# woolgathering/pyPeriod

Measured on AMD Instinct MI355X. Metric: window-projections/sec (all-p sweep, N=4096), higher is better.
Workload: dtype f64

## Files before the change

### pyperiod_amd/csrc/ph_mbest.h

```cpp
#pragma once

#include "ph_device.h"
#include "ph_pair.h"

namespace ph {

__device__ __forceinline__ bool skip_test(const uint32_t* skip, int i) { return (skip[i >> 5] >> (i & 31)) & 1u; }
__device__ __forceinline__ void skip_set(uint32_t* skip, int i) { skip[i >> 5] |= 1u << (i & 31); }

template <typename Norm>
__device__ __forceinline__ bool mbest_prefers(double ss, int p, double best_ss, int bestp, int gamma, Norm&& norm) {
  bool take = bestp == 0;
  if (!take) {
    const double lhs = gamma ? ss * (double)bestp : ss;
    const double rhs = gamma ? best_ss * (double)p : best_ss;
    if (lhs > rhs * (1.0 + 1e-14)) {
      take = true;
    } else if (lhs >= rhs * (1.0 - 1e-14)) {
      const double vn = norm(ss, gamma ? p : 0);
      const double vb = norm(best_ss, gamma ? bestp : 0);
      take = vn > vb || (vn == vb && p < bestp);
    }
  }
  return take;
}

__device__ __forceinline__ int mbest_book(int& row, int bestp, double best, int p_lo, int tid, int& filled, int& repeats,
                                          double* norms, uint32_t* periods, uint32_t* skip) {
  int action;
  __syncthreads();
  if (row >= 0 && repeats < 10) {
    action = 2;
    if (tid == 0) norms[row] += best;
    repeats += 1;
  } else if (row >= 0) {
    action = 0;
    if (tid == 0) skip_set(skip, bestp - p_lo);
    repeats = 0;
  } else {
    action = 1;
    row = filled;
    if (tid == 0) {
      periods[row] = (uint32_t)bestp;
      norms[row] = best;
    }
    filled += 1;
    repeats = 0;
  }
  return action;
}

template <typename T, bool LW>
__global__ __launch_bounds__(1024) __attribute__((amdgpu_waves_per_eu(PH_STEP1_WAVES, 8))) void k_mbest_step1(const T* __restrict__ x, int N, int num, int p_lo,
                                                        int p_hi, int gamma, unsigned flags, Tables tb,
                                                        const PGeom* __restrict__ geom,
                                                        const PassPlan* __restrict__ plan, int n_pass,
                                                        T* __restrict__ gbuf, T* gwin,
                                                        int max_iters, uint32_t* __restrict__ periods_out,
                                                        double* __restrict__ norms_out, T* __restrict__ rows_out,
                                                        int row_stride, double* __restrict__ dnorm_out,
                                                        int* __restrict__ status_out,
                                                        int* __restrict__ sweeps_out, int small_means) {
  extern __shared__ __attribute__((aligned(16))) unsigned char smem[];
  Carve cv(smem);
  T* work = window_buf<T, LW>(cv, gwin, N + kPad);
  const bool general = flags & (kTrunc | kOrth);
  T* buf = !general ? nullptr : gbuf ? gbuf + (int64_t)blockIdx.x * N : cv.take<T>(N);
  double* red = cv.take<double>(kRedDoubles);
  double* wbest = cv.take<double>(kMaxWaves);
  int* wbestp = cv.take<int>(kMaxWaves);
  double* norms = cv.take<double>(num);
  uint32_t* periods = cv.take<uint32_t>(num);
  const int P = p_hi - p_lo + 1;
  uint32_t* skip = cv.take<uint32_t>((P + 31) / 32);
  T* msm = small_means ? cv.take<T>(kPairSmallP) : nullptr;
  T* prt = small_means ? cv.take<T>(kPairSplitW) : nullptr;

  const int64_t w = blockIdx.x;
  const int tid = threadIdx.x;
  const int lane = tid & (kWave - 1);
  const int wv = __builtin_amdgcn_readfirstlane(tid >> 6);
  const int nw = blockDim.x >> 6;
  T* rows = rows_out + w * (int64_t)num * row_stride;

  load_window(x + w * (int64_t)N, work, N);
  zero_pad(work, N);
  for (int k = tid; k < num; k += blockDim.x) {
    norms[k] = 0.0;
    periods[k] = 0u;
  }
  for (int k = tid; k < (P + 31) / 32; k += blockDim.x) skip[k] = 0u;
  __syncthreads();
  const double data_norm = uniform_f64(periodic_norm_from_sq(block_sumsq(work, N, red), N, 0));

  int filled = 0;
  int repeats = 0;
  int status = 0;
  int iters = 0;
  while (filled < num) {
    if (++iters > max_iters) {
      status = 2;
      break;
    }
    double best = 0.0;
    int bestp = 0;
    if (!general) {
      double best_ss = 0.0;
      wave_sweep_plan<T, LW>(work, N, geom, plan, wv, n_pass, nw, lane, [&](double ss, int p) {
        if (skip_test(skip, p - p_lo) || !(ss > 0.0)) return;
        bool take = bestp == 0;
        if (!take) {
          const double lhs = gamma ? ss * (double)bestp : ss;
          const double rhs = gamma ? best_ss * (double)p : best_ss;
          if (lhs > rhs * (1.0 + 1e-14)) {
            take = true;
          } else if (lhs >= rhs * (1.0 - 1e-14)) {
            const double vn = periodic_norm_from_sq(ss, N, gamma ? p : 0);
            const double vb = periodic_norm_from_sq(best_ss, N, gamma ? bestp : 0);
            take = vn > vb || (vn == vb && p < bestp);
          }
        }
        if (take) {
          best_ss = ss;
          bestp = p;
        }
      });
      best = bestp != 0 ? periodic_norm_from_sq(best_ss, N, gamma ? bestp : 0) : 0.0;
      if (!(best > 0.0)) bestp = 0;
      wave_argmax(best, bestp);
      if (lane == 0) {
        wbest[wv] = best;
        wbestp[wv] = bestp;
      }
      __syncthreads();
      red_argmax(wbest, wbestp, nw, best, bestp);
      __syncthreads();
    } else {
      for (int p = p_lo; p <= p_hi; ++p) {
        const double v = block_sweep_value(work, buf, N, p, gamma ? p : 0, flags, tb, red);
        if (v > best && !skip_test(skip, p - p_lo)) {
          best = v;
          bestp = p;
        }
      }
    }
    if (bestp == 0) {
      status = 1;
      break;
    }
    int row = -1;
    for (int k = 0; k < num; ++k)
      if (periods[k] == (uint32_t)bestp) row = k;
    int action;
    __syncthreads();
    if (row >= 0 && repeats < 10) {
      action = 2;
      if (tid == 0) norms[row] += best;
      repeats += 1;
    } else if (row >= 0) {
      action = 0;
      if (tid == 0) skip_set(skip, bestp - p_lo);
      repeats = 0;
    } else {
      action = 1;
      row = filled;
      if (tid == 0) {
        periods[row] = (uint32_t)bestp;
        norms[row] = best;
      }
      filled += 1;
      repeats = 0;
    }
    T* brow = rows + (int64_t)(row < 0 ? 0 : row) * row_stride;
    if (!general && msm && bestp <= kPairSmallP) {
      split_row_means(work, msm, prt, N, bestp, tid, min((int)blockDim.x, kPairSplitW));
      if (tid < bestp) {
        const T m = msm[tid];
        if (action == 1)
          brow[tid] = m;
        else if (action == 2)
          brow[tid] += m;
      }
      int idx = tid % bestp;
      const int step = blockDim.x % bestp;
      for (int n = tid; n < N; n += blockDim.x) {
        work[n] -= msm[idx];
        idx += step;
        idx = idx >= bestp ? idx - bestp : idx;
      }
    } else if (!general) {
      const Fold f(N, bestp);
      for (int j = tid; j < bestp; j += blockDim.x) {
        const T m = residue_mean(work, f, j, false);
        const int cnt = f.count(j);
        if (action == 1)
          brow[j] = m;
        else if (action == 2)
          brow[j] += m;
        for (int r = 0; r < cnt; ++r) work[r * bestp + j] -= m;
      }
    } else {
      project_lds(work, buf, N, bestp, flags, tb);
      for (int n = tid; n < N; n += blockDim.x) {
        const T m = buf[n];
        if (n < bestp) {
          if (action == 1)
            brow[n] = m;
          else if (action == 2)
            brow[n] += m;
        }
        work[n] -= m;
      }
    }
    __syncthreads();
  }
  __syncthreads();
  for (int k = tid; k < num; k += blockDim.x) {
    periods_out[w * num + k] = periods[k];
    norms_out[w * num + k] = norms[k];
  }
  if (tid == 0) {
    dnorm_out[w] = data_norm;
    status_out[w] = status;
    if (sweeps_out) sweeps_out[w] = status == 2 ? iters - 1 : iters;
  }
}

constexpr int kPairCoop = 6;

enum {
  MP_LISTED = 0,
  MP_FILLED = 2,
  MP_REPEATS = 4,
  MP_STATUS = 6,
  MP_SWEEPS = 8,
  MP_RUNNING = 10,
  MP_EXACT_ALL = 12,
  MP_QUEUE = 14,
  MP_WORDS = 16
};
enum { MP_UNIT = 0, MP_SCALE = 2, MP_DOUBLES = 4 };

__device__ __forceinline__ double pair_exact_part(const double* __restrict__ xs, int p, const PGeom& g, int first, int stride) {
  double part = 0.0;
  for (int j = first; j < p; j += stride) {
    const bool full = j < g.nfull;
    const double s = column_sum(xs, j, p, full ? g.rows : g.rows - 1);
    part = fma(s * s, full ? g.w_full : g.w_short, part);
  }
  return part;
}

__global__ __launch_bounds__(1024) __attribute__((amdgpu_waves_per_eu(PH_STEP1_WAVES, 8))) void k_mbest_step1_pair(
    const double* __restrict__ x, int W, int N, int num, int p_lo, int p_hi, int p_scr, int gamma,
    const int* __restrict__ fac_off, const int* __restrict__ fac_q, const PGeom* __restrict__ geom, const PGeomF* __restrict__ geomf, const double* __restrict__ radq, const PassPlan* __restrict__ plan, int n_pass,
    double* __restrict__ gres, int max_iters, uint32_t* __restrict__ periods_out, double* __restrict__ norms_out,
    double* __restrict__ rows_out, int row_stride, double* __restrict__ dnorm_out, int* __restrict__ status_out,
    int* __restrict__ sweeps_out) {
  extern __shared__ __attribute__((aligned(16))) unsigned char smem[];
  Carve cv(smem);
  f2* pw = cv.take<f2>(N + kPad);
  double* stg = cv.take<double>(N + kPad);
  double* red = cv.take<double>(kRedDoubles);
  double* wbest = cv.take<double>(kMaxWaves);
  int* wbestp = cv.take<int>(kMaxWaves);
  double* norms = cv.take<double>(2 * num);
  uint32_t* periods = cv.take<uint32_t>(2 * num);
  const int P = p_hi - p_lo + 1;
  const int SK = (P + 31) / 32;
  uint32_t* skip = cv.take<uint32_t>(2 * SK);
  int* list = cv.take<int>(2 * kPairListCap);
  int* ctl = cv.take<int>(MP_WORDS);
  double* dst2 = cv.take<double>(MP_DOUBLES);
  double* msm = cv.take<double>(kPairSmallP);
  double* prt = cv.take<double>(kPairSplitW);

  const int tid = threadIdx.x;
  const int wv = __builtin_amdgcn_readfirstlane(tid >> 6);
  const int nw = blockDim.x >> 6;
  const size_t gstride = win_stride((size_t)N);
  float* pwf = reinterpret_cast<float*>(pw);
  const double sqrtN = uniform_f64(sqrt((double)N));

  for (int k = tid; k < 2 * num; k += blockDim.x) {
    norms[k] = 0.0;
    periods[k] = 0u;
  }
  for (int k = tid; k < 2 * SK; k += blockDim.x) skip[k] = 0u;
  if (tid < MP_WORDS) ctl[tid] = tid == MP_QUEUE ? nw : 0;
  zero_pad(stg, N);
  for (int i = tid; i < kPad; i += blockDim.x) pw[N + i] = f2_zero();
  for (int w = 0; w < 2; ++w) {
    const int64_t gw = 2 * (int64_t)blockIdx.x + w;
    const bool exists = gw < W;
    __syncthreads();
    if (exists) {
      load_window(x + gw * (int64_t)N, stg, N);
    } else {
      for (int n = tid; n < N; n += blockDim.x) stg[n] = 0.0;
    }
    __syncthreads();
    const double rsq = block_sumsq(stg, N, red);
    const double sc = uniform_f64(pair_pick_scale(rsq, N));
    for (int n = tid; n < N; n += blockDim.x) pwf[2 * n + w] = (float)(stg[n] * sc);
    if (tid == 0) {
      dst2[MP_UNIT + w] = rsq * sc * sc * (1.0 + 1e-9);
      dst2[MP_SCALE + w] = sc;
      ctl[MP_RUNNING + w] = exists ? 1 : 0;
      ctl[MP_EXACT_ALL + w] = pair_usable(rsq) ? 0 : 1;
      if (exists) dnorm_out[gw] = periodic_norm_from_sq_n(rsq, sqrtN, 0);
    }
  }
  StageClock<kPairTimers, 5, 2> clk;
  WgStamp<kClocks> stamp;
  for (;;) {
    __syncthreads();
    const bool act0 = __builtin_amdgcn_readfirstlane(ctl[MP_RUNNING]) != 0, act1 = __builtin_amdgcn_readfirstlane(ctl[MP_RUNNING + 1]) != 0;
    if (!act0 && !act1) break;
    prio_by_progress(__builtin_amdgcn_readfirstlane(max(ctl[MP_SWEEPS], ctl[MP_SWEEPS + 1])));
    if (wv == 0 && pair_lane() == 0) ctl[MP_LISTED] = ctl[MP_LISTED + 1] = 0;
    f2* vals = reinterpret_cast<f2*>(stg);
    pair_sweep_plan<false, true>(
        pw, N, geomf, plan, wv, n_pass, nw, [&](float z, int q) { pair_store1(vals, z, q, p_lo); },
        [&](float z, int q_a, int q_b) { pair_store2(vals, z, q_a, q_b, p_lo); },
        PH_PAIR_QUEUE ? &ctl[MP_QUEUE] : nullptr);
    __syncthreads();
    clk.mark(0);
    prio_short_phase();
    {
    const int tid = (wv << 6) + pair_lane();
    const int lane = tid & (kWave - 1);
    if (tid == 0) ctl[MP_QUEUE] = nw;
    {
      const bool scr0 = act0 && !__builtin_amdgcn_readfirstlane(ctl[MP_EXACT_ALL]), scr1 = act1 && !__builtin_amdgcn_readfirstlane(ctl[MP_EXACT_ALL + 1]);
      if (scr0 || scr1) {
        const double unit0 = uniform_f64(dst2[MP_UNIT]), unit1 = uniform_f64(dst2[MP_UNIT + 1]);
        const int i0 = p_scr - p_lo;
        const bool cover = i0 > 0;
        const int SD = (i0 + 31) >> 5;
        uint32_t* seen = reinterpret_cast<uint32_t*>(stg);
        for (int k = tid; k < 2 * SD; k += blockDim.x) seen[k] = 0u;
        const double slack = cover ? pair_cover_slack(N) : 0.0;
        struct Entry {
          f2 v;
          double rad, rq;
          bool skip0, skip1;
        };
        auto entry = [&](int idx) {
          Entry e;
          const int q = p_lo + idx;
          const uint32_t bit = 1u << (idx & 31);
          e.v = vals[idx];
          e.rad = radq[q];
          e.rq = gamma ? 1.0 / (double)q : 1.0;
          e.skip0 = (skip[idx >> 5] & bit) != 0;
          e.skip1 = (skip[SK + (idx >> 5)] & bit) != 0;
          return e;
        };
        const int idx_own = i0 + tid;
        Entry own = {f2_zero(), 0.0, 1.0, true, true};
        if (idx_own < P) own = entry(idx_own);
        double lo0 = -1.0 / 0.0, lo1 = -1.0 / 0.0;
        for (int idx = idx_own; idx < P; idx += blockDim.x) {
          const Entry e = idx == idx_own ? own : entry(idx);
          double a = (double)e.v.x - e.rad * unit0, b = (double)e.v.y - e.rad * unit1;
          if (gamma) {
            a *= e.rq;
            b *= e.rq;
          }
          if (!e.skip0 && a > lo0) lo0 = a;
          if (!e.skip1 && b > lo1) lo1 = b;
        }
        lo0 = wave_max(lo0);
        lo1 = wave_max(lo1);
        if (lane == 0) {
          red[wv] = lo0;
          red[kMaxWaves + wv] = lo1;
        }
        __syncthreads();
        lo0 = uniform_f64(red_combine<true>(red, nw));
        lo1 = uniform_f64(red_combine<true>(red + kMaxWaves, nw));
        const bool none0 = cover && scr0 && !(lo0 > -1.0 / 0.0), none1 = cover && scr1 && !(lo1 > -1.0 / 0.0);
        if (tid == 0 && none0) ctl[MP_LISTED] = kPairListCap + 1;
        if (tid == 0 && none1) ctl[MP_LISTED + 1] = kPairListCap + 1;
        const double thr0 = lo0 - fabs(lo0) * 1e-9, thr1 = lo1 - fabs(lo1) * 1e-9;
        for (int idx = idx_own; idx < P; idx += blockDim.x) {
          const Entry e = idx == idx_own ? own : entry(idx);
          const int q = p_lo + idx;
          const double rad = e.rad + slack;
          double a = (double)e.v.x + rad * unit0, b = (double)e.v.y + rad * unit1;
          if (gamma) {
            a *= e.rq;
            b *= e.rq;
          }
          const bool hit0 = scr0 && !none0 && a >= thr0, hit1 = scr1 && !none1 && b >= thr1;
          if (hit0 && !e.skip0) {
            const int k = atomicAdd(&ctl[MP_LISTED], 1);
            if (k < kPairListCap) list[k] = q;
          }
          if (hit1 && !e.skip1) {
            const int k = atomicAdd(&ctl[MP_LISTED + 1], 1);
            if (k < kPairListCap) list[kPairListCap + k] = q;
          }
          if (cover && (hit0 || hit1)) {
            const int f1 = fac_off[q + 1];
            for (int f = fac_off[q] - (p_lo == 1 ? 1 : 0); f < f1; ++f) {
              const int d = f < fac_off[q] ? 1 : fac_q[f];
              if (d < p_lo || d >= p_scr) continue;
              const int di = d - p_lo;
              const uint32_t dbit = 1u << (di & 31);
              for (int w = 0; w < 2; ++w) {
                if (!(w ? hit1 : hit0) || (skip[w * SK + (di >> 5)] & dbit)) continue;
                if (atomicOr(&seen[w * SD + (di >> 5)], dbit) & dbit) continue;
                const int k = atomicAdd(&ctl[MP_LISTED + w], 1);
                if (k < kPairListCap) list[w * kPairListCap + k] = d;
              }
            }
          }
        }
      }
    }
    __syncthreads();
    clk.mark(1);
    for (int w = 0; w < 2; ++w) {
      if (!(w ? act1 : act0)) continue;
      const int64_t gw = 2 * (int64_t)blockIdx.x + w;
      int filled = __builtin_amdgcn_readfirstlane(ctl[MP_FILLED + w]), repeats = __builtin_amdgcn_readfirstlane(ctl[MP_REPEATS + w]), status = 0,
          iters = __builtin_amdgcn_readfirstlane(ctl[MP_SWEEPS + w]);
      const int nlisted = __builtin_amdgcn_readfirstlane(ctl[MP_LISTED + w]);
      const bool exact_all = __builtin_amdgcn_readfirstlane(ctl[MP_EXACT_ALL + w]) != 0 || nlisted > kPairListCap;
      int ncand = exact_all ? P : nlisted;
      double* nrm = norms + w * num;
      uint32_t* per = periods + w * num;
      uint32_t* sk = skip + w * SK;
      const int* lst = list + w * kPairListCap;
      __syncthreads();
      if (iters + 1 > max_iters) {
        status = 2;
      } else {
        const double* src = iters == 0 ? x + gw * (int64_t)N : gres + gw * gstride;
        iters += 1;
        load_window(src, stg, N);
        __syncthreads();
        clk.mark(2);
        if (kPairTimers) {
          clk.count(0, ncand);
          clk.count(1, exact_all ? 1 : 0);
        }
        if (p_scr > p_lo && !exact_all && ncand > 1) {
          for (int k = wv; k < ncand; k += nw) {
            const int p = lst[k];
            const PGeom g = geom[p];
            const double part = p < 64 ? wave_partial_small(stg, N, p, g, lane) : pair_exact_part(stg, p, g, lane, kWave);
            const double ss = wave_sum(part);
            if (lane == 0) msm[k] = ss;
          }
          __syncthreads();
          if (wv == 0) {
            const int k0 = lane, k1 = kWave + lane;
            const double v0 = k0 < ncand ? msm[k0] : -1.0, v1 = k1 < ncand ? msm[k1] : -1.0;
            const int q0 = lst[k0], q1 = k1 < kPairListCap ? lst[k1] : 0;
            const double top = wave_max(fmax(v0, v1));
            const bool keep0 = k0 < ncand && v0 >= top - fabs(top) * 1e-9, keep1 = k1 < ncand && v1 >= top - fabs(top) * 1e-9;
            const unsigned long long m0 = __ballot(keep0), m1 = __ballot(keep1);
            const unsigned long long below = (1ull << lane) - 1ull;
            const int n0 = __popcll(m0);
            int* out = list + w * kPairListCap;
            if (keep0) out[__popcll(m0 & below)] = q0;
            if (keep1) out[n0 + __popcll(m1 & below)] = q1;
            if (lane == 0) ctl[MP_LISTED + w] = n0 + __popcll(m1);
          }
          __syncthreads();
          ncand = __builtin_amdgcn_readfirstlane(ctl[MP_LISTED + w]);
        }
        double best_ss = 0.0;
        int bestp = 0;
        const auto norm = [&](double s, int div) { return periodic_norm_from_sq_n(s, sqrtN, div); };
        auto consider = [&](double ss, int p) {
          if (!(ss > 0.0)) return;
          if (mbest_prefers(ss, p, best_ss, bestp, gamma, norm)) {
            best_ss = ss;
            bestp = p;
          }
        };
        double best = 0.0;
        if (ncand <= kPairCoop) {
          for (int k = 0; k < ncand; ++k) {
            const int p = exact_all ? p_lo + k : lst[k];
            if (skip_test(sk, p - p_lo)) continue;
            const PGeom g = geom[p];
            double part = 0.0;
            if (p < 64) {
              if (wv == 0) part = wave_partial_small(stg, N, p, g, lane);
            } else {
              part = pair_exact_part(stg, p, g, tid, blockDim.x);
            }
            consider(block_sum(part, red), p);
          }
          best = bestp != 0 ? periodic_norm_from_sq_n(best_ss, sqrtN, gamma ? bestp : 0) : 0.0;
          if (!(best > 0.0)) bestp = 0;
        } else {
          for (int k = wv; k < ncand; k += nw) {
            const int p = exact_all ? p_lo + k : lst[k];
            if (skip_test(sk, p - p_lo)) continue;
            const PGeom g = geom[p];
            const double part = p < 64 ? wave_partial_small(stg, N, p, g, lane) : pair_exact_part(stg, p, g, lane, kWave);
            consider(wave_sum(part), p);
          }
          best = bestp != 0 ? periodic_norm_from_sq_n(best_ss, sqrtN, gamma ? bestp : 0) : 0.0;
          if (!(best > 0.0)) bestp = 0;
          if (lane == 0) {
            wbest[wv] = best;
            wbestp[wv] = bestp;
          }
          __syncthreads();
          red_argmax(wbest, wbestp, nw, best, bestp);
          __syncthreads();
        }
        clk.mark(3);
        if (bestp == 0) {
          status = 1;
        } else {
          int row = -1;
          for (int k0 = 0; k0 < num; k0 += kWave) {
            const unsigned long long hit = __ballot(k0 + lane < num && per[k0 + lane] == (uint32_t)bestp);
            if (hit) row = k0 + 63 - __clzll(hit);
          }
          const int action = mbest_book(row, bestp, best, p_lo, tid, filled, repeats, nrm, per, sk);
          double* brow = rows_out + (gw * (int64_t)num + (row < 0 ? 0 : row)) * row_stride;
          const bool more = filled < num;
          const double sc = uniform_f64(dst2[MP_SCALE + w]);
          double* dst = gres + gw * gstride;
          double acc = 0.0;
          const PGeom gb = geom[__builtin_amdgcn_readfirstlane(bestp)];
          const Fold f(bestp, gb.rows, gb.nfull);
          if (bestp <= kPairSmallP) {
            split_row_means(stg, msm, prt, N, bestp, tid, kPairSplitW);
            if (tid < bestp) {
              const double m = msm[tid];
              if (action == 1)
                brow[tid] = m;
              else if (action == 2)
                brow[tid] += m;
            }
            if (more) {
              int idx = tid % bestp;
              const int step = blockDim.x % bestp;
              for (int n = tid; n < N; n += blockDim.x) {
                const double v = stg[n] - msm[idx];
                dst[n] = v;
                pwf[2 * n + w] = (float)(v * sc);
                acc = fma(v, v, acc);
                idx += step;
                idx = idx >= bestp ? idx - bestp : idx;
              }
            }
          } else {
            for (int j = tid; j < bestp; j += blockDim.x) {
              const double m = residue_mean(stg, f, j, false);
              const int cnt = f.count(j);
              if (action == 1)
                brow[j] = m;
              else if (action == 2)
                brow[j] += m;
              if (more) {
                for (int r = 0; r < cnt; ++r) {
                  const int n = r * bestp + j;
                  const double v = stg[n] - m;
                  dst[n] = v;
                  pwf[2 * n + w] = (float)(v * sc);
                  acc = fma(v, v, acc);
                }
              }
            }
          }
          if (more) {
            const double rsq = block_sum(acc, red);
            const double unit = rsq * sc * sc;
            const bool ok = pair_usable(rsq);
            if (pair_image_stale(rsq, sc, N)) {
              const double sc2 = uniform_f64(pair_pick_scale(rsq, N));
              __syncthreads();
              pair_rescale(pwf, w, N, (float)(sc2 / sc), tid);
              if (tid == 0) {
                dst2[MP_UNIT + w] = rsq * sc2 * sc2 * (1.0 + 1e-9);
                dst2[MP_SCALE + w] = sc2;
              }
            } else if (tid == 0) {
              dst2[MP_UNIT + w] = unit * (1.0 + 1e-9);
            }
            if (tid == 0) ctl[MP_EXACT_ALL + w] = ok ? 0 : 1;
          }
        }
      }
      __syncthreads();
      if (tid == 0) {
        ctl[MP_FILLED + w] = filled;
        ctl[MP_REPEATS + w] = repeats;
        ctl[MP_STATUS + w] = status;
        ctl[MP_SWEEPS + w] = iters;
        ctl[MP_RUNNING + w] = (status == 0 && filled < num) ? 1 : 0;
      }
      clk.mark(4);
    }
    }
  }
  if (kClocks && (blockIdx.x % 16) == 7 && tid == 0) {
    stamp.finish();
    printf("PAIRWG %d start %lld end %lld cycles %lld MHz %.0f hwid %x xcc %x\n", (int)blockIdx.x, stamp.wk0, stamp.wk1, stamp.ck1 - stamp.ck0,
           100.0 * (double)(stamp.ck1 - stamp.ck0) / (double)(stamp.wk1 - stamp.wk0), stamp.hwid, stamp.xcc);
  }
  if (kPairTimers && blockIdx.x < PH_PAIR_TIMERS_WGS && tid == 0)
    printf("pair timers (100 MHz ticks) screen %lld scan %lld load %lld exact %lld update %lld  candidates %d exact_all %d sweeps %d %d\n",
           clk.ticks(0), clk.ticks(1), clk.ticks(2), clk.ticks(3), clk.ticks(4), clk.counted(0), clk.counted(1), ctl[MP_SWEEPS], ctl[MP_SWEEPS + 1]);
  __syncthreads();
  for (int w = 0; w < 2; ++w) {
    const int64_t gw = 2 * (int64_t)blockIdx.x + w;
    if (gw >= W) continue;
    for (int k = tid; k < num; k += blockDim.x) {
      periods_out[gw * num + k] = periods[w * num + k];
      norms_out[gw * num + k] = norms[w * num + k];
    }
    if (tid == 0) {
      status_out[gw] = ctl[MP_STATUS + w];
      if (sweeps_out) sweeps_out[gw] = ctl[MP_SWEEPS + w];
    }
  }
}

__device__ __forceinline__ PGeom make_geom(int N, int p) {
  const int rows = (N + p - 1) / p;
  PGeom g;
  g.rows = rows;
  g.nfull = p - (rows * p - N);
  g.w_full = 1.0 / (double)rows;
  g.w_short = rows > 1 ? 1.0 / (double)(rows - 1) : 0.0;
  return g;
}

constexpr int kStep2Pre = 3;
typedef __attribute__((address_space(3))) void* lds_void_ptr;
typedef const __attribute__((address_space(1))) void* global_void_ptr;

template <typename T>
__device__ __forceinline__ void expand_row(const T* __restrict__ src, int p, T* __restrict__ dst, int N) {
  const int step = blockDim.x % p;
  int idx = threadIdx.x % p;
  for (int n = threadIdx.x; n < N; n += blockDim.x) {
    dst[n] = src[idx];
    idx += step;
    if (idx >= p) idx -= p;
  }
}

template <typename T, bool LW>
__global__ __launch_bounds__(kBlockWide) __attribute__((amdgpu_waves_per_eu(PH_STEP1_WAVES, 8))) void k_mbest_step2(int N, int num, int gamma, int stale_p, unsigned flags,
                                                        Tables tb, const PGeom* __restrict__ geom, int max_fac,
                                                        T* __restrict__ gbuf, T* gwin,
                                                        uint32_t* __restrict__ periods_io,
                                                        double* __restrict__ norms_io, T* __restrict__ bases_out,
                                                        const double* __restrict__ dnorm,
                                                        const int* __restrict__ status, T* __restrict__ rows_io,
                                                        int row_stride) {
  extern __shared__ __attribute__((aligned(16))) unsigned char smem[];
  Carve cv(smem);
  T* rowbuf = window_buf<T, LW>(cv, gwin, N + kPad);
  T* buf = gbuf ? gbuf + (int64_t)blockIdx.x * N : cv.take<T>(N);
  double* red = cv.take<double>(kRedDoubles);
  double* norms = cv.take<double>(num);
  uint32_t* periods = cv.take<uint32_t>(num);
  double* fvals = cv.take<double>(max_fac > 0 ? max_fac : 1);
  int* ffac = cv.take<int>(max_fac > 0 ? max_fac : 1);
  PGeom* fgeom = cv.take<PGeom>(kMaxWaves);
  int* fa = cv.take<int>(num);
  int* fb = cv.take<int>(num);
  int* slot = cv.take<int>(num);
  int* ffac_next = cv.take<int>(max_fac > 64 ? max_fac : 64);

  const int64_t w = blockIdx.x;
  const int tid = threadIdx.x;
  const int lane = tid & (kWave - 1);
  const int wv = __builtin_amdgcn_readfirstlane(tid >> 6);
  const int nw = blockDim.x >> 6;
  const bool general = flags & (kTrunc | kOrth);
  const bool periodic_rows = sizeof(T) == 8 && !general;
  T* rows = rows_io + w * (int64_t)num * row_stride;
  for (int k = tid; k < num; k += blockDim.x) {
    norms[k] = norms_io[w * num + k];
    const uint32_t per = periods_io[w * num + k];
    periods[k] = per;
    fa[k] = tb.fac_off[per];
    fb[k] = tb.fac_off[per + 1];
    slot[k] = k;
  }
  zero_pad(rowbuf, N);
  __syncthreads();

  StageClock<kStep2Timers, 6, 2> clk;
  const int gdiv = gamma ? stale_p : 0;
  int i = (status[w] == 0) ? 0 : num;
  auto next_row = [&](int r) {
    while (r < num && fa[r] == fb[r]) ++r;
    return r;
  };
  const T* stage = nullptr;
  int stage_row = -1;
  T* out = bases_out + w * (int64_t)num * N;
  int done = 0;
  auto flush_rows = [&](int upto) {
    for (; done < upto; ++done) {
      const int pr = (int)periods[done];
      T* dst = out + (int64_t)done * N;
      if (pr == 0) {
        for (int n = tid; n < N; n += blockDim.x) dst[n] = T(0);
      } else {
        expand_row(rows + (int64_t)slot[done] * row_stride, pr, dst, N);
      }
    }
  };
  i = next_row(i);
  clk.mark(0);
  while (i < num) {
    const int per = (int)periods[i];
    const int a = fa[i], b = fb[i];
    const T* src = rows + (int64_t)slot[i] * row_stride;
    const int zend = per + (per >> 1) + 256;
    const bool short_row = periodic_rows && zend <= N + kPad;
    if (short_row) {
      const PGeom gp = make_geom(N, per);
      const double cf = (double)gp.rows, cs = (double)(gp.rows - 1);
      if (stage_row == i) {
        double t[kStep2Pre];
#pragma unroll
        for (int u = 0; u < kStep2Pre; ++u) {
          const int k = tid + u * blockDim.x;
          t[u] = k < per ? (double)stage[k] : 0.0;
        }
        __syncthreads();
#pragma unroll
        for (int u = 0; u < kStep2Pre; ++u) {
          const int k = tid + u * blockDim.x;
          if (k < zend) rowbuf[k] = (T)(t[u] * (k < gp.nfull ? cf : cs));
        }
        for (int k = tid + kStep2Pre * blockDim.x; k < zend; k += blockDim.x) rowbuf[k] = T(0);
        if (tid < b - a) ffac[tid] = ffac_next[tid];
      } else {
        for (int k = tid; k < zend; k += blockDim.x)
          rowbuf[k] = (T)(k < per ? (double)src[k] * (k < gp.nfull ? cf : cs) : 0.0);
        if (tid < b - a) ffac[tid] = tb.fac_q[a + tid];
      }
    } else {
      expand_row(src, per, rowbuf, N);
      if (!general && tid < b - a) ffac[tid] = tb.fac_q[a + tid];
    }
    __syncthreads();
    clk.mark(1);
    const int inext = next_row(i + 1);
    stage_row = -1;
    if (LW && short_row && inext < num) {
      const int pn = (int)periods[inext];
      const int so = (zend + 1) & ~1;
      const int npieces = (pn + 127) >> 7;
      if (pn <= kStep2Pre * (int)blockDim.x && pn + (pn >> 1) + 256 <= N + kPad && so + 128 * npieces <= N &&
          128 * npieces <= row_stride && fb[inext] - fa[inext] <= 64) {
        const T* srcn = rows + (int64_t)slot[inext] * row_stride;
        for (int j = wv; j < npieces; j += nw)
          __builtin_amdgcn_global_load_lds((global_void_ptr)(srcn + 128 * j + 2 * lane),
                                           (lds_void_ptr)(rowbuf + so + 128 * j), 16, 0, 0);
        if (wv == nw - 1)
          __builtin_amdgcn_global_load_lds((global_void_ptr)(tb.fac_q + fa[inext] + lane), (lds_void_ptr)ffac_next, 4, 0, 0);
        stage = rowbuf + so;
        stage_row = inext;
      }
    }
    double top = 0.0, last = 0.0;
    int topf = -1;
    if (!general) {
      for (int k = wv; k < b - a; k += nw) {
        const int f = ffac[k];
        if (lane == 0) {
          PGeom g;
          if (short_row) {
            g = make_geom(N, f);
            g.rows = per / f + 1;
          } else {
            g = geom[f];
          }
          fgeom[wv] = g;
        }
        ram_wave_sync();
        const double ss = wave_sum(wave_partial<T, false, LW>(rowbuf, short_row ? per : N, f, fgeom[wv], lane));
        ram_wave_sync();
        if (lane == 0) fvals[k] = periodic_norm_from_sq(ss, N, gdiv);
      }
      clk.mark(2);
      __builtin_amdgcn_s_waitcnt(0x0F70);
      __syncthreads();
      clk.mark(3);
      flush_rows(i);
      for (int k = 0; k < b - a; ++k) {
        const double v = fvals[k];
        if (v > top) {
          top = v;
          topf = ffac[k];
        }
        last = v;
      }
    } else {
      flush_rows(i);
      for (int k = a; k < b; ++k) {
        const int f = tb.fac_q[k];
        const double v = block_sweep_value(rowbuf, buf, N, f, gdiv, flags, tb, red);
        if (v > top) {
          top = v;
          topf = f;
        }
        last = v;
      }
    }
    bool split = false;
    if (topf >= 0) {
      bool present = false;
      for (int k = 0; k < num; ++k) present |= (periods[k] == (uint32_t)topf);
      if (!present) {
        double floor_q = norms[0];
        for (int k = 1; k < num; ++k) floor_q = fmin(floor_q, norms[k]);
        split = (last + top) > (norms[num - 1] + norms[i]) && last > floor_q && top > floor_q;
      }
    }
    const int s_here = slot[i], s_last = slot[num - 1];
    __syncthreads();
    clk.mark(4);
    clk.count(0);
    clk.count(1, split ? 1 : 0);
    if (!split) {
      i = inext;
      continue;
    }
    stage_row = -1;
    if (short_row) {
      expand_row(src, per, rowbuf, N);
      __syncthreads();
    }
    project_lds(rowbuf, buf, N, topf, flags, tb);
    {
      T* dst = rows + (int64_t)s_last * row_stride;
      if (i + 1 < num) {
        T* rem = rows + (int64_t)s_here * row_stride;
        for (int k = tid; k < per; k += blockDim.x) rem[k] = rowbuf[k] - buf[k];
      }
      for (int k = tid; k < topf; k += blockDim.x) dst[k] = buf[k];
    }
    if (tid == 0) {
      for (int r = num - 1; r >= i + 2; --r) {
        norms[r] = norms[r - 1];
        periods[r] = periods[r - 1];
        fa[r] = fa[r - 1];
        fb[r] = fb[r - 1];
        slot[r] = slot[r - 1];
      }
      if (i + 1 < num) {
        norms[i + 1] = last;
        periods[i + 1] = (uint32_t)per;
        fa[i + 1] = a;
        fb[i + 1] = b;
        slot[i + 1] = s_here;
      }
      norms[i] = top;
      periods[i] = (uint32_t)topf;
      fa[i] = tb.fac_off[topf];
      fb[i] = tb.fac_off[topf + 1];
      slot[i] = s_last;
    }
    __threadfence_block();
    __syncthreads();
    i = next_row(i);
  }
  __syncthreads();
  flush_rows(num);
  clk.mark(5);
  if (kStep2Timers && (blockIdx.x % 128) == 5 && tid == 0)
    printf("step2 wg %d (100 MHz ticks): init %lld stage %lld folds %lld dma+barrier %lld flush+scan %lld rest(split,final flush) %lld total %lld rows %d splits %d\n",
           (int)blockIdx.x, clk.ticks(0), clk.ticks(1), clk.ticks(2), clk.ticks(3), clk.ticks(4), clk.ticks(5), clk.total(), clk.counted(0), clk.counted(1));
  const double dn = dnorm[w];
  for (int k = tid; k < num; k += blockDim.x) {
    periods_io[w * num + k] = periods[k];
    norms_io[w * num + k] = norms[k] / dn;
  }
}

}
```

Measured before the change: 9.911 billion.

## Defer basis output tiling to end with vectorized double-buffered stores and direct fold projection

Removes the incremental flush of expanded basis rows inside the split loop and instead writes all rows once at the end, using 16-byte vector stores with a two-batch software pipeline and separate handling of misaligned edges. The periodic split path now computes residue means directly per fold position instead of calling the general projection, and LDS row expansion is batched. This aims to cut scattered scalar global writes and per-iteration overhead, at the cost of more registers and code complexity.

Result: no change. 9.989 billion, median of 3 (+0.8%).

```diff
diff --git a/pyperiod_amd/csrc/ph_mbest.h b/pyperiod_amd/csrc/ph_mbest.h
--- a/pyperiod_amd/csrc/ph_mbest.h
+++ b/pyperiod_amd/csrc/ph_mbest.h
@@ -653,6 +653,115 @@
   }
 }
 
+template <typename T>
+__device__ __forceinline__ void expand_row_lds(const T* __restrict__ src, int p, T* rowbuf, int N, int tid) {
+  const int nt = blockDim.x;
+  for (int k0 = tid; k0 < p; k0 += 8 * nt) {
+    T t[8];
+#pragma unroll
+    for (int u = 0; u < 8; ++u) t[u] = src[min(k0 + u * nt, p - 1)];
+#pragma unroll
+    for (int u = 0; u < 8; ++u)
+      if (k0 + u * nt < p) rowbuf[k0 + u * nt] = t[u];
+  }
+  __syncthreads();
+  const int step = nt % p;
+  int idx = tid % p;
+  for (int n0 = p + tid; n0 < N; n0 += 4 * nt) {
+    T t[4];
+#pragma unroll
+    for (int u = 0; u < 4; ++u) {
+      t[u] = rowbuf[idx];
+      idx += step;
+      if (idx >= p) idx -= p;
+    }
+#pragma unroll
+    for (int u = 0; u < 4; ++u)
+      if (n0 + u * nt < N) rowbuf[n0 + u * nt] = t[u];
+  }
+}
+
+constexpr int kTileU = 4;
+
+template <typename T>
+struct TileBatch {
+  static constexpr int V = 16 / sizeof(T);
+  using vec_t = typename std::conditional<sizeof(T) == 8, double2, float4>::type;
+  vec_t* body;
+  int nchunks;
+  int c0;
+  T v[kTileU][V];
+
+  __device__ __forceinline__ void load(const T* __restrict__ src, int p, T* dst, int N, int b, int tid) {
+    const int nt = blockDim.x;
+    const int mis = (int)((reinterpret_cast<uintptr_t>(dst) / sizeof(T)) & (V - 1));
+    const int h = min((V - mis) & (V - 1), N);
+    body = reinterpret_cast<vec_t*>(dst + h);
+    nchunks = (N - h) / V;
+    c0 = b * kTileU * nt + tid;
+    if (p == 0) {
+#pragma unroll
+      for (int u = 0; u < kTileU; ++u)
+#pragma unroll
+        for (int e = 0; e < V; ++e) v[u][e] = T(0);
+      return;
+    }
+    const int step = (V * nt) % p;
+    int i0 = (int)(((unsigned)h + (unsigned)c0 * V) % (unsigned)p);
+#pragma unroll
+    for (int u = 0; u < kTileU; ++u) {
+      int i = i0;
+#pragma unroll
+      for (int e = 0; e < V; ++e) {
+        v[u][e] = src[i];
+        i += 1;
+        if (i >= p) i = 0;
+      }
+      i0 += step;
+      if (i0 >= p) i0 -= p;
+    }
+  }
+  __device__ __forceinline__ void settle() {
+#pragma unroll
+    for (int u = 0; u < kTileU; ++u)
+#pragma unroll
+      for (int e = 0; e < V; ++e) asm volatile("" : "+v"(v[u][e]));
+  }
+  __device__ __forceinline__ void store() {
+    settle();
+#pragma unroll
+    for (int u = 0; u < kTileU; ++u) {
+      const int c = c0 + u * (int)blockDim.x;
+      if (c < nchunks) {
+        vec_t q;
+        q.x = v[u][0];
+        q.y = v[u][1];
+        if constexpr (V == 4) {
+          q.z = v[u][2];
+          q.w = v[u][3];
+        }
+        body[c] = q;
+      }
+    }
+  }
+};
+
+template <typename T>
+__device__ __forceinline__ void tile_edges(const T* __restrict__ rows, int row_stride, const int* slot, const uint32_t* periods, T* out, int N, int num, int tid) {
+  constexpr int V = 16 / sizeof(T), E = 2 * (V - 1);
+  for (int k = tid; k < num * E; k += blockDim.x) {
+    const int r = k / E, e = k - r * E;
+    T* dst = out + (int64_t)r * N;
+    const int mis = (int)((reinterpret_cast<uintptr_t>(dst) / sizeof(T)) & (V - 1));
+    const int h = min((V - mis) & (V - 1), N);
+    const int tail = (N - h) % V;
+    if (e >= h + tail) continue;
+    const int n = e < h ? e : N - tail + (e - h);
+    const int p = (int)periods[r];
+    dst[n] = p ? rows[(int64_t)slot[r] * row_stride + n % p] : T(0);
+  }
+}
+
 template <typename T, bool LW>
 __global__ __launch_bounds__(kBlockWide) __attribute__((amdgpu_waves_per_eu(PH_STEP1_WAVES, 8))) void k_mbest_step2(int N, int num, int gamma, int stale_p, unsigned flags,
                                                         Tables tb, const PGeom* __restrict__ geom, int max_fac,
@@ -679,7 +788,6 @@
 
   const int64_t w = blockIdx.x;
   const int tid = threadIdx.x;
-  const int lane = tid & (kWave - 1);
   const int wv = __builtin_amdgcn_readfirstlane(tid >> 6);
   const int nw = blockDim.x >> 6;
   const bool general = flags & (kTrunc | kOrth);
@@ -696,7 +804,7 @@
   zero_pad(rowbuf, N);
   __syncthreads();
 
-  StageClock<kStep2Timers, 6, 2> clk;
+  StageClock<kStep2Timers, 7, 2> clk;
   const int gdiv = gamma ? stale_p : 0;
   int i = (status[w] == 0) ? 0 : num;
   auto next_row = [&](int r) {
@@ -705,22 +813,11 @@
   };
   const T* stage = nullptr;
   int stage_row = -1;
-  T* out = bases_out + w * (int64_t)num * N;
-  int done = 0;
-  auto flush_rows = [&](int upto) {
-    for (; done < upto; ++done) {
-      const int pr = (int)periods[done];
-      T* dst = out + (int64_t)done * N;
-      if (pr == 0) {
-        for (int n = tid; n < N; n += blockDim.x) dst[n] = T(0);
-      } else {
-        expand_row(rows + (int64_t)slot[done] * row_stride, pr, dst, N);
-      }
-    }
-  };
   i = next_row(i);
   clk.mark(0);
   while (i < num) {
+    const int lane = pair_lane();
+    const int tid = (wv << 6) + lane;
     const int per = (int)periods[i];
     const int a = fa[i], b = fb[i];
     const T* src = rows + (int64_t)slot[i] * row_stride;
@@ -797,7 +894,6 @@
       __builtin_amdgcn_s_waitcnt(0x0F70);
       __syncthreads();
       clk.mark(3);
-      flush_rows(i);
       for (int k = 0; k < b - a; ++k) {
         const double v = fvals[k];
         if (v > top) {
@@ -807,7 +903,6 @@
         last = v;
       }
     } else {
-      flush_rows(i);
       for (int k = a; k < b; ++k) {
         const int f = tb.fac_q[k];
         const double v = block_sweep_value(rowbuf, buf, N, f, gdiv, flags, tb, red);
@@ -838,17 +933,28 @@
       continue;
     }
     stage_row = -1;
+    const int tid_s = (wv << 6) + pair_lane();
     if (short_row) {
-      expand_row(src, per, rowbuf, N);
+      if constexpr (LW)
+        expand_row_lds(src, per, rowbuf, N, tid_s);
+      else
+        expand_row(src, per, rowbuf, N);
       __syncthreads();
     }
-    project_lds(rowbuf, buf, N, topf, flags, tb);
-    {
-      T* dst = rows + (int64_t)s_last * row_stride;
-      if (i + 1 < num) {
-        T* rem = rows + (int64_t)s_here * row_stride;
+    T* dst = rows + (int64_t)s_last * row_stride;
+    T* rem = i + 1 < num ? rows + (int64_t)s_here * row_stride : nullptr;
+    if (!general) {
+      const Fold f(N, topf);
+      for (int j = tid_s; j < topf; j += blockDim.x) {
+        const T m = residue_mean(rowbuf, f, j, false);
+        dst[j] = m;
+        if (rem)
+          for (int k = j; k < per; k += topf) rem[k] = rowbuf[k] - m;
+      }
+    } else {
+      project_lds(rowbuf, buf, N, topf, flags, tb);
+      if (rem)
         for (int k = tid; k < per; k += blockDim.x) rem[k] = rowbuf[k] - buf[k];
-      }
       for (int k = tid; k < topf; k += blockDim.x) dst[k] = buf[k];
     }
     if (tid == 0) {
@@ -874,14 +980,35 @@
     }
     __threadfence_block();
     __syncthreads();
+    clk.mark(5);
     i = next_row(i);
   }
   __syncthreads();
-  flush_rows(num);
-  clk.mark(5);
+  {
+    T* out = bases_out + w * (int64_t)num * N;
+    constexpr int V = TileBatch<T>::V;
+    const int nb = max(1, (N / V + kTileU * (int)blockDim.x - 1) / (kTileU * (int)blockDim.x));
+    const int tid = (wv << 6) + pair_lane();
+    auto load = [&](TileBatch<T>& t, int item) {
+      const int r = item / nb;
+      t.load(rows + (int64_t)slot[r] * row_stride, (int)periods[r], out + (int64_t)r * N, N, item - r * nb, tid);
+    };
+    tile_edges(rows, row_stride, slot, periods, out, N, num, tid);
+    const int items = num * nb;
+    TileBatch<T> ta, tb2;
+    load(ta, 0);
+    for (int item = 0; item < items; item += 2) {
+      if (item + 1 < items) load(tb2, item + 1);
+      ta.store();
+      if (item + 1 >= items) break;
+      if (item + 2 < items) load(ta, item + 2);
+      tb2.store();
+    }
+  }
+  clk.mark(6);
   if (kStep2Timers && (blockIdx.x % 128) == 5 && tid == 0)
-    printf("step2 wg %d (100 MHz ticks): init %lld stage %lld folds %lld dma+barrier %lld flush+scan %lld rest(split,final flush) %lld total %lld rows %d splits %d\n",
-           (int)blockIdx.x, clk.ticks(0), clk.ticks(1), clk.ticks(2), clk.ticks(3), clk.ticks(4), clk.ticks(5), clk.total(), clk.counted(0), clk.counted(1));
+    printf("step2 wg %d (100 MHz ticks): init %lld stage %lld folds %lld dma+barrier %lld scan %lld split %lld tile-out %lld total %lld rows %d splits %d\n",
+           (int)blockIdx.x, clk.ticks(0), clk.ticks(1), clk.ticks(2), clk.ticks(3), clk.ticks(4), clk.ticks(5), clk.ticks(6), clk.total(), clk.counted(0), clk.counted(1));
   const double dn = dnorm[w];
   for (int k = tid; k < num; k += blockDim.x) {
     periods_io[w * num + k] = periods[k];
```
